# DMDung2k3/Intelligent-Video-Analysis-Retrieval-System

Measured on AMD Instinct MI355X. Metric: frames/s embedded (+ query-vs-index cosine pairs/s; top-10 recall vs CPU ref), higher is better.
Workload: dtype bf16; 1 GPU; BASELINE configs[1]: ViT-B/32 bf16 random-init embed of 224x224 RGB frames + 1M-row x 512-d fp32 index cosine top-10 (per GPU); frames_total=299008, index_rows_per_gpu=1000000, queries=10, k=10, parallelism=1 x (frames + index rows sharded per GPU); one all-gather of (score,id) + merge

## Files before the change

### intelligent-video-analysis-retrieval-system_amd/csrc/tower.hip

```cpp
#include "tower.h"
#include "tower_kernels.h"

#include <cmath>
#include <cstring>
#include <vector>

extern "C" {

int ivr_tower_create(ivr_ctx *ctx, const ivr_tower_desc *d, ivr_tower **out) {
    IVR_REQUIRE(ctx && d && out, "ivr_tower_create: NULL argument");
    IVR_REQUIRE(d->kind == IVR_KIND_VISION || d->kind == IVR_KIND_TEXT, "ivr_tower_create: kind=%d", d->kind);
    IVR_REQUIRE(d->width >= 64 && d->width % 64 == 0 && d->width <= 2048, "ivr_tower_create: width=%d must be a multiple of 64 in [64,2048]",
                d->width);
    IVR_REQUIRE(d->heads >= 1 && d->heads <= 32 && d->width == d->heads * 64, "ivr_tower_create: head_dim must be 64 (width=%d heads=%d)",
                d->width, d->heads);
    IVR_REQUIRE(d->mlp >= 64 && d->mlp % 64 == 0, "ivr_tower_create: mlp=%d must be a multiple of 64", d->mlp);
    IVR_REQUIRE(d->layers >= 1 && d->layers <= 64, "ivr_tower_create: layers=%d", d->layers);
    IVR_REQUIRE(d->tokens >= 1 && d->tokens <= 1024, "ivr_tower_create: tokens=%d", d->tokens);
    IVR_REQUIRE(d->out_dim >= 0 && d->out_dim % 16 == 0 && d->out_dim <= 2048, "ivr_tower_create: out_dim=%d", d->out_dim);
    IVR_REQUIRE(d->act == IVR_ACT_QUICK_GELU || d->act == IVR_ACT_GELU_ERF, "ivr_tower_create: act=%d", d->act);
    IVR_REQUIRE(d->compute == IVR_COMPUTE_BF16 || d->compute == IVR_COMPUTE_F32 || d->compute == IVR_COMPUTE_FP8,
                "ivr_tower_create: compute=%d", d->compute);
    IVR_REQUIRE(d->compute != IVR_COMPUTE_FP8 || (d->width % 128 == 0 && d->mlp % 128 == 0),
                "ivr_tower_create: the fp8 mode needs width and mlp to be multiples of 128 (width=%d mlp=%d)", d->width, d->mlp);
// ... 164 lines not shown
int layer_gemm(ivr_tower *t, bool site_fp8, int epi, GemmArgs &g, const std::string &wname, hipStream_t s) {
    if (site_fp8) {
        g.W = wptr<void>(t, wname + "@e4m3");
        g.colscale = wptr<float>(t, wname + "@scale");
        return ivr_launch_gemm_fp8(epi, g, s);
    }
    g.W = wptr<void>(t, wname);
    return ivr_launch_gemm(t->d.compute == IVR_COMPUTE_F32, epi, g, s);
}

int env_zigzag() {
    static const int v = [] {
        const char *e = getenv("IVR_ZIGZAG");
        return e ? (atoi(e) != 0) : 1;
    }();
    return v;
}

bool env_prune_last() {
    const char *e = getenv("IVR_PRUNE_LAST");
    return e ? (atoi(e) != 0) : true;
}

int run_layers(ivr_tower *t, int n, int T, bool prune_last, hipStream_t s) {
    const ivr_tower_desc &d = t->d;
    const bool f32 = d.compute == IVR_COMPUTE_F32;

    auto kind = [&](bool site8) { return f32 ? OUT_F32 : site8 ? OUT_FP8 : OUT_BF16; };
    const int D = d.width, rows = n * T;
    const int zz = env_zigzag();
    int rc;
    for (int i = 0; i < d.layers; ++i) {
        const std::string p = "l" + std::to_string(i) + ".";
        const int sites = i >= d.fp8_first_layer ? t->sites : 0;
        const bool q8 = sites & IVR_FP8_SITE_QKV, o8 = sites & IVR_FP8_SITE_ATTN_OUT, f18 = sites & IVR_FP8_SITE_FC1, f28 = sites & IVR_FP8_SITE_FC2;
        const bool mlp_cls = t->mlp_cls && (f18 || f28);
        const bool last = prune_last && i == d.layers - 1;
        if (t->debug_out && t->debug_layer == i)
            IVR_HIP(hipMemcpyAsync(t->debug_out, t->resid, (size_t)rows * D * 4, hipMemcpyDeviceToDevice, s));
        rc = ivr_launch_layernorm(kind(q8), t->resid, 1, nullptr, wptr<float>(t, p + "ln1_g"), wptr<float>(t, p + "ln1_b"), d.ln_eps,
                                  t->xn, rows, D, s, zz);
        if (rc) return rc;
        GemmArgs g;
        int att_ld = D;
        if (!f32 && !q8 && ivr_fused_qkv_attention_ok(rows, T, D, d.heads, d.causal)) {
            rc = ivr_launch_qkv_attention(t->xn, wptr<void>(t, p + "qkv_w"), wptr<float>(t, p + "qkv_b"), t->att, n, T, D, d.heads, o8, s, 0,
                                          last);
            if (rc) return rc;
        } else {
            if (last) att_ld = T * D;
            g.A = t->xn;
            g.lda = D;
            g.ldw = D;
            g.M = rows;
            g.N = 3 * D;
            g.K = D;
            g.bias = wptr<float>(t, p + "qkv_b");
            g.out = t->qkv;
            g.ldo = 3 * D;
            g.tag = "gemm_qkv";
            rc = layer_gemm(t, q8, EPI_STORE, g, p + "qkv_w", s);
            if (rc) return rc;
            rc = ivr_launch_attention(f32, t->qkv, t->att, n, T, D, d.heads, d.causal, s, o8);
            if (rc) return rc;
        }
        g = GemmArgs();
        g.A = t->att;
        g.lda = att_ld;
        g.ldw = D;
        g.M = last ? n : rows;
// ... 288 lines not shown
    IVR_HIP(hipSetDevice(t->ctx->device));
    hipStream_t s = (hipStream_t)stream;
    const bool f32 = d.compute == IVR_COMPUTE_F32;
    const int D = d.width, T = d.tokens, G2 = T - 1;
    int rc = ivr_launch_vision_cls(t->resid, wptr<float>(t, "cls"), wptr<float>(t, "pos"), n, T, D, s);
    if (rc) return rc;
    GemmArgs g;
    g.A = patches;
    g.lda = t->kpad;
    g.W = wptr<void>(t, "patch_w");
    g.ldw = t->kpad;
    g.M = n * G2;
    g.N = D;
    g.K = t->kpad;
    g.bias = d.patch_bias ? wptr<float>(t, "patch_b") : nullptr;
    g.resid = t->resid;
    g.ldr = D;
    g.pos = wptr<float>(t, "pos");
    g.T = T;
    g.G2 = G2;
    g.tag = "gemm_patch";
    rc = ivr_launch_gemm(f32, EPI_PATCH, g, s);
    if (rc) return rc;
    if (d.pre_ln) {
        rc = ivr_launch_layernorm(OUT_F32, t->resid, 1, nullptr, wptr<float>(t, "pre_ln_g"), wptr<float>(t, "pre_ln_b"), d.ln_eps, t->resid,
                                  n * T, D, s);
        if (rc) return rc;
    }
    const bool prune = env_prune_last() && !(t->debug_out && t->debug_layer == d.layers);
    rc = run_layers(t, n, T, prune, s);
    if (rc) return rc;
    return run_pool(t, n, T, nullptr, normalize, out, s);
}

int ivr_tower_encode_text(ivr_tower *t, const int64_t *ids, int q, int T, int normalize, float *out, ivr_stream stream) {
    IVR_REQUIRE(t && (q == 0 || (ids && out)), "ivr_tower_encode_text: NULL argument");
    std::lock_guard<std::mutex> lk(t->mu);
    if (!t->finalized) return ivr_fail(IVR_ERR_STATE, "ivr_tower_encode_text: tower not finalized");
    const ivr_tower_desc &d = t->d;
    IVR_REQUIRE(d.kind == IVR_KIND_TEXT, "ivr_tower_encode_text: not a text tower");
    IVR_REQUIRE(T >= 1 && T <= d.tokens, "ivr_tower_encode_text: T=%d outside [1,%d]", T, d.tokens);
    IVR_REQUIRE(q >= 0 && (int64_t)q * T <= (int64_t)t->max_batch * d.tokens && q <= t->max_batch,
                "ivr_tower_encode_text: q=%d exceeds max_batch=%d", q, t->max_batch);
    if (q == 0) return IVR_OK;
    IVR_HIP(hipSetDevice(t->ctx->device));
    hipStream_t s = (hipStream_t)stream;
    int rc = ivr_launch_text_embed(t->resid, ids, wptr<float>(t, "tok"), wptr<float>(t, "pos"), q, T, d.width, d.vocab, d.eos_id,
                                   t->eos_pos, s);
    if (rc) return rc;
    rc = run_layers(t, q, T, false, s);
    if (rc) return rc;
    return run_pool(t, q, T, t->eos_pos, normalize, out, s);
}
// ... 188 lines not shown
```

### intelligent-video-analysis-retrieval-system_amd/csrc/tower_kernels.h

```cpp
#pragma once
#include "ivr_common.h"

enum { EPI_STORE = 0, EPI_RESID = 1, EPI_PATCH = 2, EPI_F32 = 3 };

struct GemmArgs {
    const void *A = nullptr;
    int lda = 0;
    const void *W = nullptr;
    int ldw = 0;
    int M = 0, N = 0, K = 0;
    const float *bias = nullptr;
    void *out = nullptr;
    int ldo = 0;
    float *resid = nullptr;
    int ldr = 0;
    const float *pos = nullptr;
    int T = 0, G2 = 0;
    int act = -1;
    const char *tag = nullptr;
    int group_m = 8;
    const float *colscale = nullptr;
    int out8 = 0;
    int wide_epi = 0;
    int reverse_m = 0;
    int stagger = 0;
    int skip_mod = 0;
};

int ivr_launch_gemm(bool f32, int epi, const GemmArgs &g, hipStream_t s);
int ivr_launch_gemm_fp8(int epi, const GemmArgs &g, hipStream_t s);
enum { OUT_BF16 = 0, OUT_F32 = 1, OUT_FP8 = 2 };
int ivr_launch_layernorm(int out_kind, const float *x, int row_mul, const int *offs, const float *g, const float *b, float eps,
                         void *out, int rows, int D, hipStream_t s, int reverse = 0);
int ivr_launch_attention(bool f32, const void *qkv, void *att, int n, int T, int D, int heads, int causal, hipStream_t s,
                         bool out_fp8 = false);
bool ivr_fused_qkv_attention_shape_ok(int M, int T, int D, int heads, int causal);
bool ivr_fused_qkv_attention_ok(int M, int T, int D, int heads, int causal);
int ivr_launch_qkv_attention(const void *xn, const void *w, const float *bias, void *att, int n, int T, int D, int heads, bool out_fp8,
                             hipStream_t s, int reverse = 0, int pooled = 0);
int ivr_launch_vision_cls(float *resid, const float *cls, const float *pos, int n, int T, int D, hipStream_t s);
int ivr_launch_text_embed(float *resid, const int64_t *ids, const float *tok, const float *pos, int q, int T, int D, int vocab,
                          int eos, int *eos_pos, hipStream_t s);
int ivr_launch_bf16_to_e4m3(const void *src, void *dst, int64_t count, hipStream_t s);
int ivr_launch_f_normalize(const float *x, float *out, int n, int d, int normalize, hipStream_t s);
```

### intelligent-video-analysis-retrieval-system_amd/csrc/tower_kernels.hip

```cpp
#include "tower.h"
#include "tower_kernels.h"

#include <map>
#include <mutex>
#include <type_traits>

#include <algorithm>
#include <cstdlib>

namespace {

template <typename T>
struct El;
template <>
struct El<unsigned short> {
    static __device__ __forceinline__ void unpack(const uint4 &u, float (&f)[8]) {
        f[0] = __uint_as_float(u.x << 16);
        f[1] = __uint_as_float(u.x & 0xffff0000u);
        f[2] = __uint_as_float(u.y << 16);
        f[3] = __uint_as_float(u.y & 0xffff0000u);
        f[4] = __uint_as_float(u.z << 16);
        f[5] = __uint_as_float(u.z & 0xffff0000u);
        f[6] = __uint_as_float(u.w << 16);
        f[7] = __uint_as_float(u.w & 0xffff0000u);
// ... 81 lines not shown
__global__ __launch_bounds__(256) void text_embed_kernel(float *__restrict__ resid, const int64_t *__restrict__ ids,
                                                         const float *__restrict__ tok, const float *__restrict__ pos,
                                                         int T, int D, int vocab) {
    const int64_t r = blockIdx.x;
    const int t = (int)(r % T);
    int64_t id = ids[r];
    id = id < 0 ? 0 : (id >= vocab ? vocab - 1 : id);
    const float *e = tok + id * D;
    for (int k = threadIdx.x; k < D; k += blockDim.x) resid[r * D + k] = e[k] + pos[(int64_t)t * D + k];
}

__global__ void eos_pos_kernel(const int64_t *__restrict__ ids, int q, int T, int eos, int *__restrict__ out) {
    const int r = blockIdx.x * blockDim.x + threadIdx.x;
    if (r >= q) return;
    int p = 0;
    for (int t = 0; t < T; ++t)
        if (ids[(int64_t)r * T + t] == eos) {
            p = t;
            break;
        }
    out[r] = p;
}

template <typename TOut>
__global__ __launch_bounds__(256) void layernorm_kernel(const float *__restrict__ x, int row_mul, const int *__restrict__ offs,
                                                        const float *__restrict__ g, const float *__restrict__ b, float eps,
                                                        TOut *__restrict__ out, int rows, int D, int reverse) {
    const int lane = threadIdx.x & 63;
    int row = blockIdx.x * 4 + (threadIdx.x >> 6);
    if (row >= rows) return;
    if (reverse) row = rows - 1 - row;
    const int64_t srow = (int64_t)row * row_mul + (offs ? offs[row] : 0);
    const float4 *src = reinterpret_cast<const float4 *>(x + srow * D);
    const int nv = D >> 2;
    float4 v[8];
#pragma unroll
    for (int i = 0; i < 8; ++i) {
        const int idx = lane + 64 * i;
        v[i] = make_float4(0.f, 0.f, 0.f, 0.f);
        if (idx < nv) v[i] = src[idx];
    }
    const float x0 = __shfl(v[0].x, 0, 64);
    float s = 0.f;
#pragma unroll
    for (int i = 0; i < 8; ++i) {
        const int idx = lane + 64 * i;
        if (idx < nv) {
            v[i].x -= x0;
            v[i].y -= x0;
            v[i].z -= x0;
            v[i].w -= x0;
            s += (v[i].x + v[i].y) + (v[i].z + v[i].w);
        }
    }
    const float mean = ivr_wave_sum(s) / (float)D;
    float ss = 0.f;
#pragma unroll
    for (int i = 0; i < 8; ++i) {
        const int idx = lane + 64 * i;
        if (idx < nv) {
            const float a = v[i].x - mean, bb = v[i].y - mean, c = v[i].z - mean, d = v[i].w - mean;
            ss += (a * a + bb * bb) + (c * c + d * d);
        }
    }
    const float rstd = 1.0f / sqrtf(ivr_wave_sum(ss) / (float)D + eps);
    TOut *orow = out + (int64_t)row * D;
#pragma unroll
    for (int i = 0; i < 8; ++i) {
        const int idx = lane + 64 * i;
        if (idx < nv) {
            const float4 gg = reinterpret_cast<const float4 *>(g)[idx], bv = reinterpret_cast<const float4 *>(b)[idx];
            float y[4];
            y[0] = (v[i].x - mean) * rstd * gg.x + bv.x;
            y[1] = (v[i].y - mean) * rstd * gg.y + bv.y;
            y[2] = (v[i].z - mean) * rstd * gg.z + bv.z;
            y[3] = (v[i].w - mean) * rstd * gg.w + bv.w;
            El<TOut>::store4(orow + idx * 4, y);
        }
    }
}

__global__ __launch_bounds__(256) void f_normalize_kernel(const float *__restrict__ x, float *__restrict__ out, int n, int d,
                                                          int normalize) {
    const int lane = threadIdx.x & 63;
    const int row = blockIdx.x * 4 + (threadIdx.x >> 6);
    if (row >= n) return;
    const float *p = x + (int64_t)row * d;
    float ss = 0.f;
// ... 1235 lines not shown
                                 : "v"(offV[nt]));
                else
                    asm volatile("ds_read_b64_tr_b16 %0, %2 offset:4096\n\tds_read_b64_tr_b16 %1, %2 offset:6144\n\ts_waitcnt lgkmcnt(0)"
                                 : "=&v"(lo), "=&v"(hi)
                                 : "v"(offV[nt]));
                const uint4 vf = make_uint4(lo.x, lo.y, hi.x, hi.y);
                o = __builtin_amdgcn_mfma_f32_16x16x32_bf16(__builtin_bit_cast(bf16x8_t, vf), __builtin_bit_cast(bf16x8_t, pf[ks]), o, 0, 0, 0);
            }
            if (q < Tn) {
                const float v[4] = {o[0] * inv, o[1] * inv, o[2] * inv, o[3] * inv};
                El<TOut>::store4(op + nt * 16, v);
            }
        }
    }
}

struct QkvAttnArgs {
    const void *X = nullptr;
    const void *W = nullptr;
    const float *bias = nullptr;
    void *att = nullptr;
    int M = 0, D = 0, T = 0, heads = 0, G = 0, group_m = 4, reverse = 0;
    int pooled = 0;
};

constexpr int QA_WBYTES = 192 * ROWB;
constexpr int QA_LDS = 3 * LX_BYTES + 2 * QA_WBYTES;
constexpr int QP_LDS = 160 * 1024;
constexpr int QA_REGION = 264 * ROWB;

template <typename TOut, bool PERS>
__device__ __forceinline__ void qkv_attn_body(const QkvAttnArgs &g, unsigned char *smem) {
    typedef __bf16 bf16x8_t __attribute__((ext_vector_type(8)));
    typedef unsigned short T;
    if constexpr (!PERS) { IVR_STAMP(0) }
    const int tid = threadIdx.x, lane = tid & 63;
    const int wave = __builtin_amdgcn_readfirstlane(tid >> 6);
    const int wm = wave >> 2, wn = wave & 3;
    const int RT = g.G * g.T;
    const int MT = (g.M + RT - 1) / RT, NT = g.heads;
    const int xcd = blockIdx.x & 7, slot = blockIdx.x >> 3, nslots = gridDim.x >> 3;
    const int nitems = xcd_panels(MT, xcd) * NT;
    if (slot >= nitems) return;
    const int count = PERS ? (nitems - slot + nslots - 1) / nslots : 1;
    auto locate = [&](int n, int &tm_, int &h_) { xcd_tile(slot + n * nslots, xcd, MT, NT, g.group_m, g.reverse, tm_, h_); };
    const int KT = g.D / 64;
    const unsigned lds0 = (unsigned)(size_t)smem;

    unsigned voffX[4], voffW;
    {
        const int c = (lane & 7) ^ (lane >> 3);
#pragma unroll
        for (int j = 0; j < 4; ++j) voffX[j] = (unsigned)((8 * (wave * 4 + j) + (lane >> 3)) * g.D) * 2u + c * 16;
        voffW = (unsigned)((lane >> 3) * g.D) * 2u + c * 16;
    }
    auto item_offsets = [&](int tm_, int h_, unsigned &sx, unsigned (&sw)[3]) {
        sx = (unsigned)(tm_ * RT) * (unsigned)g.D * 2u;
#pragma unroll
        for (int j = 0; j < 3; ++j) {
            const int p = wave * 3 + j;
            sw[j] = (unsigned)(((p >> 3) * g.D + h_ * 64 + 8 * (p & 7)) * g.D) * 2u;
        }
    };
    const auto rsX = __builtin_amdgcn_make_buffer_rsrc(const_cast<void *>(g.X), 0, (int)((int64_t)g.M * g.D * 2), 0x00020000);
    const auto rsW = __builtin_amdgcn_make_buffer_rsrc(const_cast<void *>(g.W), 0, (int)((int64_t)3 * g.D * g.D * 2), 0x00020000);
    auto xbase = [](int xs) { return PERS ? (xs == 0 ? 0 : xs == 1 ? 57344 : 90112) : xs * LX_BYTES; };
    auto wbase = [](int b) { return PERS ? (b ? 122880 : 32768) : 3 * LX_BYTES + b * QA_WBYTES; };
    constexpr int IMG = PERS ? 62464 : 0;
    static_assert(IMG + 3 * QA_REGION <= (PERS ? QP_LDS : QA_LDS), "Q | K | V images past the end of the LDS");
    auto piece = [&](unsigned sx, const unsigned (&sw)[3], int kt, int xs, int j) {
        const unsigned adv = (unsigned)kt * ROWB;
        if (j < 4)
            __builtin_amdgcn_raw_ptr_buffer_load_lds(rsX, (__attribute__((address_space(3))) void *)(smem + xbase(xs) + (wave * 4 + j) * 1024), 16,
                                                     voffX[j], sx + adv, 0, 0);
        else
            __builtin_amdgcn_raw_ptr_buffer_load_lds(rsW, (__attribute__((address_space(3))) void *)(smem + wbase(kt & 1) + (wave * 3 + j - 4) * 1024),
                                                     16, voffW, sw[j - 4] + adv, 0, 0);
    };
    unsigned foX[2], foW[2];
#pragma unroll
    for (int kk = 0; kk < 2; ++kk) {
        const unsigned f = (lane & 15) * ROWB + ((((kk << 2) + (lane >> 4)) ^ (lane & 7)) << 4);
        foX[kk] = lds0 + (wm * 128) * ROWB + f;
        foW[kk] = lds0 + (wn * 48) * ROWB + f;
    }

    int tm, h;
    locate(0, tm, h);
    unsigned sx0, swW[3];
    item_offsets(tm, h, sx0, swW);
#define QA_ROW(XF, WF, MTI)                                                                                \
    _Pragma("unroll") for (int nt = 0; nt < 3; ++nt) mma_chunk<T>(WF[nt], XF[MTI], acc[nt][MTI]);          \
    __builtin_amdgcn_sched_barrier(0);
#define QA_RD3(DST, ADDR)                                                                                  \
    asm volatile("ds_read_b128 %0, %1" : "=v"(DST[0]) : "v"(ADDR));                                         \
    asm volatile("ds_read_b128 %0, %1 offset:2048" : "=v"(DST[1]) : "v"(ADDR));                             \
    asm volatile("ds_read_b128 %0, %1 offset:4096" : "=v"(DST[2]) : "v"(ADDR));

    u32x4 xa0[8], wa0[3], xa1[8], wa1[3];
    u32x4 *x0lo = xa0, *x0hi = xa0 + 4, *x1lo = xa1, *x1hi = xa1 + 4;
#pragma unroll
    for (int j = 0; j < 7; ++j) piece(sx0, swW, 0, 0, j);
  for (int n = 0; n < count; ++n) {
    const int m0 = tm * RT;
    f32x4 acc[3][8];
#pragma unroll
    for (int a = 0; a < 3; ++a)
#pragma unroll
        for (int b = 0; b < 8; ++b) acc[a][b] = f32x4{0.f, 0.f, 0.f, 0.f};
    float4 bq[3];
#pragma unroll
    for (int nt = 0; nt < 3; ++nt) {
        const int col = wn * 48 + nt * 16 + 4 * (lane >> 4);
        bq[nt] = *reinterpret_cast<const float4 *>(g.bias + (col >> 6) * g.D + h * 64 + (col & 63));
    }
#pragma unroll
    for (int j = 0; j < 7; ++j) piece(sx0, swW, 1, 1, j);
#pragma unroll
    for (int j = 0; j < 4; ++j) piece(sx0, swW, 2, 2, j);
    asm volatile("s_waitcnt vmcnt(11)\n\ts_barrier" ::: "memory");
    if constexpr (!PERS) { IVR_STAMP(1) }
    QA_RD3(wa0, foW[0] + wbase(0))
    IVR_RD4(x0lo, foX[0] + xbase(0), 0)
    IVR_RD4(x0hi, foX[0] + xbase(0), 8192)
    int xs = 0;
    for (int kt = 0; kt < KT; ++kt) {
        const int xs1 = xs == 2 ? 0 : xs + 1;
        const unsigned xoff = xbase(xs), woff = wbase(kt & 1), nxoff = xbase(xs1), nwoff = wbase((kt + 1) & 1);
        const bool tail = kt >= 1 && kt + 2 < KT;
        const bool morew = kt + 2 < KT, morex = kt + 3 < KT, next = kt + 1 < KT;
        const unsigned wa = foW[1] + woff, xa = foX[1] + xoff, nwa = foW[0] + nwoff, nxa = foX[0] + nxoff;
        IVR_LGKM(4)
        QA_ROW(xa0, wa0, 0)
        if (tail) piece(sx0, swW, kt + 2, xs1 == 2 ? 0 : xs1 + 1, 2);
        QA_ROW(xa0, wa0, 1)
        QA_RD3(wa1, wa)
        QA_ROW(xa0, wa0, 2)
        if (tail) piece(sx0, swW, kt + 2, xs1 == 2 ? 0 : xs1 + 1, 3);
        QA_ROW(xa0, wa0, 3)
        IVR_RD4(x1lo, xa, 0)
        IVR_LGKM(7)
        QA_ROW(xa0, wa0, 4)
        QA_ROW(xa0, wa0, 5)
        IVR_RD4(x1hi, xa, 8192)
        QA_ROW(xa0, wa0, 6)
        QA_ROW(xa0, wa0, 7)
        IVR_LGKM(0)
        if (next) {
            if (kt + 2 < KT) asm volatile("s_waitcnt vmcnt(4)\n\ts_barrier" ::: "memory");
            else asm volatile("s_waitcnt vmcnt(0)\n\ts_barrier" ::: "memory");
        }
        QA_ROW(xa1, wa1, 0)
        if (morew) piece(sx0, swW, kt + 2, 0, 4);
        QA_ROW(xa1, wa1, 1)
        if (next) { QA_RD3(wa0, nwa) }
        if (morew) piece(sx0, swW, kt + 2, 0, 5);
        QA_ROW(xa1, wa1, 2)
        if (morew) piece(sx0, swW, kt + 2, 0, 6);
        QA_ROW(xa1, wa1, 3)
        if (next) { IVR_RD4(x0lo, nxa, 0) }
        QA_ROW(xa1, wa1, 4)
        if (morex) piece(sx0, swW, kt + 3, xs, 0);
        QA_ROW(xa1, wa1, 5)
        if (next) { IVR_RD4(x0hi, nxa, 8192) }
        QA_ROW(xa1, wa1, 6)
        if (morex) piece(sx0, swW, kt + 3, xs, 1);
        QA_ROW(xa1, wa1, 7)
        xs = xs1;
    }
    IVR_LGKM(0)
#undef QA_ROW
#undef QA_RD3
    if constexpr (!PERS) { IVR_STAMP(2) }
    __builtin_amdgcn_s_barrier();

    unsigned char *const qreg = smem + IMG, *const kreg = smem + IMG + QA_REGION, *const vreg = smem + IMG + 2 * QA_REGION;
    {
        const int r = lane & 15, gq = lane >> 4;
#pragma unroll
        for (int nt = 0; nt < 3; ++nt) {
            const int col = wn * 48 + nt * 16 + 4 * gq;
            const int reg3 = col >> 6, dh = col & 63, ch = dh >> 3;
            const float4 bv = bq[nt];
            unsigned char *base = smem + IMG + reg3 * QA_REGION + (dh & 7) * 2;
#pragma unroll
            for (int mt = 0; mt < 8; ++mt) {
                const int m = wm * 128 + mt * 16 + r;
                const f32x4 a = acc[nt][mt];
                uint2 o;
                o.x = ivr_pack_bf16x2(a[0] + bv.x, a[1] + bv.y);
                o.y = ivr_pack_bf16x2(a[2] + bv.z, a[3] + bv.w);
                const unsigned pos = reg3 == 2 ? (unsigned)((((ch >> 1) ^ ((m >> 1) & 3)) << 5) | ((ch & 1) << 4))
                                               : (unsigned)((ch ^ (m & 7)) << 4);
                *reinterpret_cast<uint2 *>(base + m * ROWB + pos) = o;
            }
        }
        if (tid < 128) *reinterpret_cast<uint4 *>((tid < 64 ? kreg : vreg) + 256 * ROWB + (tid & 63) * 16) = make_uint4(0u, 0u, 0u, 0u);
    }
    __syncthreads();
#ifdef IVR_GEMM_STAMPS
    if (!PERS && threadIdx.x == 0 && blockIdx.x < 16384) ivr_gemm_stamps[blockIdx.x][6] = __builtin_amdgcn_s_memtime();
#endif
    const int h_cur = h;
    if (n + 1 < count) {
        locate(n + 1, tm, h);
        item_offsets(tm, h, sx0, swW);
#pragma unroll
        for (int j = 0; j < 7; ++j) piece(sx0, swW, 0, 0, j);
    }

    const int Tn = g.T, nqt = g.pooled ? 1 : (Tn + 15) >> 4, units = g.G * nqt;
    const int gl = lane >> 4, c = lane & 15;
    constexpr float L2E = 1.4426950408889634f;
    for (int u = wave; u < units; u += 8) {
        const int img = u / nqt, qt = u - img * nqt;
        const int R0 = img * Tn;
        if (m0 + R0 >= g.M) continue;
        const int q = qt * 16 + c;
        uint4 qf[2], kf[2][4];
        uint2 vt[4][4];
        {
            const int rq = R0 + q;
            const unsigned qa = (unsigned)(size_t)qreg + rq * ROWB, qx = rq & 7;
#pragma unroll
            for (int ks = 0; ks < 2; ++ks) asm volatile("ds_read_b128 %0, %1" : "=v"(qf[ks]) : "v"(qa + (((4 * ks + gl) ^ qx) << 4)));
            const int rk = R0 + c;
            const unsigned ka = (unsigned)(size_t)kreg + rk * ROWB, kx = rk & 7;
#pragma unroll
            for (int ks = 0; ks < 2; ++ks) {
                const unsigned a0 = ka + (((4 * ks + gl) ^ kx) << 4);
                asm volatile("ds_read_b128 %0, %1" : "=v"(kf[ks][0]) : "v"(a0));
// ... 84 lines not shown
        }
    }
    if (n + 1 < count) __syncthreads();
  }
#ifdef IVR_GEMM_STAMPS
    if constexpr (!PERS) {
        asm volatile("s_waitcnt vmcnt(0)" ::: "memory");
        __syncthreads();
        IVR_STAMP(3)
    }
#endif
}

template <typename TOut>
__global__ __launch_bounds__(512, 2) void qkv_attn_kernel(QkvAttnArgs g) {
    extern __shared__ __attribute__((aligned(16))) unsigned char smem[];
    qkv_attn_body<TOut, false>(g, smem);
}

template <typename TOut>
__global__ __launch_bounds__(512, 2) void qkv_attn_pers_kernel(QkvAttnArgs g) {
    extern __shared__ __attribute__((aligned(16))) unsigned char smem[];
    qkv_attn_body<TOut, true>(g, smem);
}

template <int EPI, int ACT>
__global__ __launch_bounds__(512, 2) void gemm_pers_kernel(GemmArgs g) {
    typedef unsigned short T;
    extern __shared__ __attribute__((aligned(16))) unsigned char smem[];
    const int tid = threadIdx.x, lane = tid & 63;
    const int wave = __builtin_amdgcn_readfirstlane(tid >> 6);
    const int wm = wave >> 2, wn = wave & 3;
    const int MT = (g.M + LBM - 1) / LBM, NT = (g.N + LBN - 1) / LBN;
    const int xcd = blockIdx.x & 7, slot = blockIdx.x >> 3, nslots = gridDim.x >> 3;
    const int lx = MT > xcd ? (MT - xcd + 7) >> 3 : 0;
    const int nitems = lx * NT;
    if (slot >= nitems) return;
    const int count = (nitems - slot + nslots - 1) / nslots;
    const int KT = g.K / 64;
    const int S = count * KT;
    const unsigned lds0 = (unsigned)(size_t)smem;
    const int gm = g.group_m;
    auto locate = [&](int n, int &tm, int &tn) {
        const unsigned i = (unsigned)(slot + n * nslots);
        const unsigned per = (unsigned)(gm * NT), grp = i / per, within = i - grp * per;
        const unsigned gme = (unsigned)min(gm, lx - (int)grp * gm);
// ... 501 lines not shown
        if (g.act == IVR_ACT_GELU_ERF) return launch_gemm8_t<EPI_STORE, IVR_ACT_GELU_ERF, true>(g, s);
        return launch_gemm8_t<EPI_STORE, -1, true>(g, s);
    }
    if (g.act == IVR_ACT_QUICK_GELU) return launch_gemm8_t<EPI_STORE, IVR_ACT_QUICK_GELU, false>(g, s);
    if (g.act == IVR_ACT_GELU_ERF) return launch_gemm8_t<EPI_STORE, IVR_ACT_GELU_ERF, false>(g, s);
    return launch_gemm8_t<EPI_STORE, -1, false>(g, s);
}

bool ivr_fused_qkv_attention_shape_ok(int M, int T, int D, int heads, int causal) {
    if (T < 1 || T > 64 || causal || D % 64 != 0 || D < 192 || D > 2048 || heads != D / 64 || M < 0 || M % T != 0) return false;
    return (int64_t)M * D * 2 < 0x7fffffff && (int64_t)3 * D * D * 2 < 0x7fffffff;
}

bool ivr_fused_qkv_attention_ok(int M, int T, int D, int heads, int causal) {
    if (!ivr_fused_qkv_attention_shape_ok(M, T, D, heads, causal)) return false;
    const int mode = env_int("IVR_FUSED_QKV", -1);
    if (mode == 0) return false;
    if (mode == 1) return true;
    const int RT = (256 / T) * T;
    return (int64_t)((M + RT - 1) / RT) * heads >= 256;
}

int ivr_launch_qkv_attention(const void *xn, const void *w, const float *bias, void *att, int n, int T, int D, int heads, bool out_fp8,
                             hipStream_t s, int reverse, int pooled) {
    if (n <= 0) return IVR_OK;
    const int M = n * T;
    IVR_REQUIRE(ivr_fused_qkv_attention_shape_ok(M, T, D, heads, 0), "fused qkv+attention: unsupported shape (n=%d T=%d D=%d heads=%d)",
                n, T, D, heads);
    const auto al16 = [](const void *p) { return reinterpret_cast<uintptr_t>(p) % 16 == 0; };
    IVR_REQUIRE(al16(xn) && al16(w) && al16(bias) && al16(att), "fused qkv+attention: operands must be 16-byte aligned");
    QkvAttnArgs g;
    g.X = xn;
    g.W = w;
    g.bias = bias;
    g.att = att;
    g.M = M;
    g.D = D;
    g.T = T;
    g.heads = heads;
    g.G = 256 / T;
    g.group_m = std::max(1, env_int("IVR_QKV_GROUP_M", 4));
    g.reverse = reverse;
    g.pooled = pooled != 0;
    const int RT = g.G * T, MT = (M + RT - 1) / RT;
    IvrProf prof("gemm_qkv_attention", s, 2.0 * M * 3.0 * D * D + 4.0 * n * heads * (double)(pooled ? std::min(T, 16) : T) * T * 64);
    const int qpers = env_int("IVR_QKV_PERS", 1);
    const bool pers = qpers == 2 || (qpers == 1 && (int64_t)MT * heads >= 2 * device_cu_count());
    void (*kern)(QkvAttnArgs) = pers ? (out_fp8 ? qkv_attn_pers_kernel<unsigned char> : qkv_attn_pers_kernel<unsigned short>)
                                     : (out_fp8 ? qkv_attn_kernel<unsigned char> : qkv_attn_kernel<unsigned short>);
    const int grid = pers ? device_cu_count() / 8 * 8 : xcd_grid(MT, heads), lds = pers ? QP_LDS : QA_LDS;
    if (int rc = ivr_func_max_lds(reinterpret_cast<const void *>(kern), lds)) return rc;
    hipLaunchKernelGGL(kern, dim3(grid), dim3(512), lds, s, g);
    IVR_LAUNCH_CHECK();
    return IVR_OK;
}

int ivr_launch_layernorm(int out_kind, const float *x, int row_mul, const int *offs, const float *g, const float *b, float eps,
                         void *out, int rows, int D, hipStream_t s, int reverse) {
    if (rows <= 0) return IVR_OK;
    IVR_REQUIRE(D % 4 == 0 && D <= 2048, "layernorm: D=%d", D);
    const unsigned grid = (unsigned)ivr_ceil_div(rows, 4);
    IvrProf prof("layernorm", s, (double)rows * D * (4 + (out_kind == OUT_F32 ? 4 : out_kind == OUT_FP8 ? 1 : 2)));
    if (out_kind == OUT_F32)
        hipLaunchKernelGGL(layernorm_kernel<float>, dim3(grid), dim3(256), 0, s, x, row_mul, offs, g, b, eps, (float *)out, rows, D, reverse);
    else if (out_kind == OUT_FP8)
        hipLaunchKernelGGL(layernorm_kernel<unsigned char>, dim3(grid), dim3(256), 0, s, x, row_mul, offs, g, b, eps,
                           (unsigned char *)out, rows, D, reverse);
    else
        hipLaunchKernelGGL(layernorm_kernel<unsigned short>, dim3(grid), dim3(256), 0, s, x, row_mul, offs, g, b, eps,
                           (unsigned short *)out, rows, D, reverse);
    IVR_LAUNCH_CHECK();
    return IVR_OK;
}

int ivr_launch_attention(bool f32, const void *qkv, void *att, int n, int T, int D, int heads, int causal, hipStream_t s, bool out_fp8) {
    if (n <= 0) return IVR_OK;
    IvrProf prof("attention", s, 4.0 * n * heads * (double)T * T * 64);
    IVR_REQUIRE(!(f32 && out_fp8), "attention: e4m3 output only from the bf16 kernels");
    if (!f32 && T <= 64) {
        const int64_t items = (int64_t)n * heads;
        if (out_fp8)
            hipLaunchKernelGGL(attention_mfma_short_kernel<unsigned char>, dim3((unsigned)ivr_ceil_div(items, 4)), dim3(256), 4 * 8192,
                               s, (const unsigned short *)qkv, (unsigned char *)att, n, T, D, heads, causal);
        else
            hipLaunchKernelGGL(attention_mfma_short_kernel<unsigned short>, dim3((unsigned)ivr_ceil_div(items, 4)), dim3(256), 4 * 8192,
                               s, (const unsigned short *)qkv, (unsigned short *)att, n, T, D, heads, causal);
        IVR_LAUNCH_CHECK();
        return IVR_OK;
    }
    if (!f32) {
        const int Tp = (int)ivr_round_up(T, 32);
        const int head_env = env_int("IVR_ATTN_HEAD", 1);
        if (head_env && 2 * Tp * 128 <= 160 * 1024 && (int64_t)T * 3 * D * 2 < 0x7fffffff) {
            const int ntiles = (T + 15) / 16;
            auto go = [&](auto qc_c, auto minw_c) -> int {
// ... 126 lines not shown
```

Measured before the change: 105,300 frames/s.

## Fuse pre-LN with layer-0 LN1 and skip full Q projection in pruned last layer

Adds a chained layernorm kernel that applies pre_ln, writes the fp32 residual back in place, and then applies layer 0's ln1 to produce xn, all in one launch, so the separate pre_ln pass and its extra read of the residual go away. In the pruned last layer, only CLS-row queries are needed. A small GEMM now projects Q for just those rows, and a new NOQ variant of the fused qkv+attention kernel computes only K and V and loads the precomputed Q rows into LDS. This cuts roughly a third of the QKV GEMM work in the last layer, at the cost of an extra small GEMM launch, more kernel variants, and tighter wait counts that could be fragile.

```diff
diff --git a/intelligent-video-analysis-retrieval-system_amd/csrc/tower.hip b/intelligent-video-analysis-retrieval-system_amd/csrc/tower.hip
--- a/intelligent-video-analysis-retrieval-system_amd/csrc/tower.hip
+++ b/intelligent-video-analysis-retrieval-system_amd/csrc/tower.hip
@@ -210,7 +210,22 @@
     return e ? (atoi(e) != 0) : true;
 }
 
-int run_layers(ivr_tower *t, int n, int T, bool prune_last, hipStream_t s) {
+bool env_preln_fused() {
+    const char *e = getenv("IVR_PRELN_FUSED");
+    return e ? (atoi(e) != 0) : true;
+}
+
+bool env_last_noq() {
+    const char *e = getenv("IVR_LAST_NOQ");
+    return e ? (atoi(e) != 0) : true;
+}
+
+int site_kind(const ivr_tower *t, int layer, int bit) {
+    const int sites = layer >= t->d.fp8_first_layer ? t->sites : 0;
+    return t->d.compute == IVR_COMPUTE_F32 ? OUT_F32 : (sites & bit) ? OUT_FP8 : OUT_BF16;
+}
+
+int run_layers(ivr_tower *t, int n, int T, bool prune_last, hipStream_t s, bool ln1_done = false) {
     const ivr_tower_desc &d = t->d;
     const bool f32 = d.compute == IVR_COMPUTE_F32;
 
@@ -226,14 +241,32 @@
         const bool last = prune_last && i == d.layers - 1;
         if (t->debug_out && t->debug_layer == i)
             IVR_HIP(hipMemcpyAsync(t->debug_out, t->resid, (size_t)rows * D * 4, hipMemcpyDeviceToDevice, s));
-        rc = ivr_launch_layernorm(kind(q8), t->resid, 1, nullptr, wptr<float>(t, p + "ln1_g"), wptr<float>(t, p + "ln1_b"), d.ln_eps,
-                                  t->xn, rows, D, s, zz);
-        if (rc) return rc;
+        if (!(ln1_done && i == 0)) {
+            rc = ivr_launch_layernorm(kind(q8), t->resid, 1, nullptr, wptr<float>(t, p + "ln1_g"), wptr<float>(t, p + "ln1_b"), d.ln_eps,
+                                      t->xn, rows, D, s, zz);
+            if (rc) return rc;
+        }
         GemmArgs g;
         int att_ld = D;
         if (!f32 && !q8 && ivr_fused_qkv_attention_ok(rows, T, D, d.heads, d.causal)) {
+            const void *qrow = nullptr;
+            if (last && env_last_noq()) {
+                g.A = t->xn;
+                g.lda = T * D;
+                g.ldw = D;
+                g.M = n;
+                g.N = D;
+                g.K = D;
+                g.bias = wptr<float>(t, p + "qkv_b");
+                g.out = t->qkv;
+                g.ldo = D;
+                g.tag = "gemm_q_cls";
+                rc = layer_gemm(t, false, EPI_STORE, g, p + "qkv_w", s);
+                if (rc) return rc;
+                qrow = t->qkv;
+            }
             rc = ivr_launch_qkv_attention(t->xn, wptr<void>(t, p + "qkv_w"), wptr<float>(t, p + "qkv_b"), t->att, n, T, D, d.heads, o8, s, 0,
-                                          last);
+                                          last, qrow);
             if (rc) return rc;
         } else {
             if (last) att_ld = T * D;
@@ -568,13 +601,19 @@
     g.tag = "gemm_patch";
     rc = ivr_launch_gemm(f32, EPI_PATCH, g, s);
     if (rc) return rc;
-    if (d.pre_ln) {
+    const bool preln_fused = d.pre_ln && env_preln_fused();
+    if (preln_fused) {
+        rc = ivr_launch_layernorm2(site_kind(t, 0, IVR_FP8_SITE_QKV), t->resid, wptr<float>(t, "pre_ln_g"), wptr<float>(t, "pre_ln_b"),
+                                   d.ln_eps, wptr<float>(t, "l0.ln1_g"), wptr<float>(t, "l0.ln1_b"), d.ln_eps, t->xn, n * T, D, s,
+                                   env_zigzag());
+        if (rc) return rc;
+    } else if (d.pre_ln) {
         rc = ivr_launch_layernorm(OUT_F32, t->resid, 1, nullptr, wptr<float>(t, "pre_ln_g"), wptr<float>(t, "pre_ln_b"), d.ln_eps, t->resid,
                                   n * T, D, s);
         if (rc) return rc;
     }
     const bool prune = env_prune_last() && !(t->debug_out && t->debug_layer == d.layers);
-    rc = run_layers(t, n, T, prune, s);
+    rc = run_layers(t, n, T, prune, s, preln_fused);
     if (rc) return rc;
     return run_pool(t, n, T, nullptr, normalize, out, s);
 }
diff --git a/intelligent-video-analysis-retrieval-system_amd/csrc/tower_kernels.h b/intelligent-video-analysis-retrieval-system_amd/csrc/tower_kernels.h
--- a/intelligent-video-analysis-retrieval-system_amd/csrc/tower_kernels.h
+++ b/intelligent-video-analysis-retrieval-system_amd/csrc/tower_kernels.h
@@ -32,12 +32,14 @@
 enum { OUT_BF16 = 0, OUT_F32 = 1, OUT_FP8 = 2 };
 int ivr_launch_layernorm(int out_kind, const float *x, int row_mul, const int *offs, const float *g, const float *b, float eps,
                          void *out, int rows, int D, hipStream_t s, int reverse = 0);
+int ivr_launch_layernorm2(int out_kind, float *x, const float *g, const float *b, float eps, const float *g2, const float *b2, float eps2,
+                          void *out, int rows, int D, hipStream_t s, int reverse = 0);
 int ivr_launch_attention(bool f32, const void *qkv, void *att, int n, int T, int D, int heads, int causal, hipStream_t s,
                          bool out_fp8 = false);
 bool ivr_fused_qkv_attention_shape_ok(int M, int T, int D, int heads, int causal);
 bool ivr_fused_qkv_attention_ok(int M, int T, int D, int heads, int causal);
 int ivr_launch_qkv_attention(const void *xn, const void *w, const float *bias, void *att, int n, int T, int D, int heads, bool out_fp8,
-                             hipStream_t s, int reverse = 0, int pooled = 0);
+                             hipStream_t s, int reverse = 0, int pooled = 0, const void *qrow = nullptr);
 int ivr_launch_vision_cls(float *resid, const float *cls, const float *pos, int n, int T, int D, hipStream_t s);
 int ivr_launch_text_embed(float *resid, const int64_t *ids, const float *tok, const float *pos, int q, int T, int D, int vocab,
                           int eos, int *eos_pos, hipStream_t s);
diff --git a/intelligent-video-analysis-retrieval-system_amd/csrc/tower_kernels.hip b/intelligent-video-analysis-retrieval-system_amd/csrc/tower_kernels.hip
--- a/intelligent-video-analysis-retrieval-system_amd/csrc/tower_kernels.hip
+++ b/intelligent-video-analysis-retrieval-system_amd/csrc/tower_kernels.hip
@@ -127,10 +127,38 @@
     out[r] = p;
 }
 
-template <typename TOut>
-__global__ __launch_bounds__(256) void layernorm_kernel(const float *__restrict__ x, int row_mul, const int *__restrict__ offs,
+__device__ __forceinline__ void ln_row_stats(float4 (&v)[8], int lane, int nv, int D, float eps, float &mean, float &rstd) {
+    const float x0 = __shfl(v[0].x, 0, 64);
+    float s = 0.f;
+#pragma unroll
+    for (int i = 0; i < 8; ++i) {
+        const int idx = lane + 64 * i;
+        if (idx < nv) {
+            v[i].x -= x0;
+            v[i].y -= x0;
+            v[i].z -= x0;
+            v[i].w -= x0;
+            s += (v[i].x + v[i].y) + (v[i].z + v[i].w);
+        }
+    }
+    mean = ivr_wave_sum(s) / (float)D;
+    float ss = 0.f;
+#pragma unroll
+    for (int i = 0; i < 8; ++i) {
+        const int idx = lane + 64 * i;
+        if (idx < nv) {
+            const float a = v[i].x - mean, bb = v[i].y - mean, c = v[i].z - mean, d = v[i].w - mean;
+            ss += (a * a + bb * bb) + (c * c + d * d);
+        }
+    }
+    rstd = 1.0f / sqrtf(ivr_wave_sum(ss) / (float)D + eps);
+}
+
+template <typename TOut, bool CHAIN = false>
+__global__ __launch_bounds__(256) void layernorm_kernel(const float *x, int row_mul, const int *__restrict__ offs,
                                                         const float *__restrict__ g, const float *__restrict__ b, float eps,
-                                                        TOut *__restrict__ out, int rows, int D, int reverse) {
+                                                        float *mid, const float *__restrict__ g2, const float *__restrict__ b2,
+                                                        float eps2, TOut *__restrict__ out, int rows, int D, int reverse) {
     const int lane = threadIdx.x & 63;
     int row = blockIdx.x * 4 + (threadIdx.x >> 6);
     if (row >= rows) return;
@@ -145,30 +173,26 @@
         v[i] = make_float4(0.f, 0.f, 0.f, 0.f);
         if (idx < nv) v[i] = src[idx];
     }
-    const float x0 = __shfl(v[0].x, 0, 64);
-    float s = 0.f;
-#pragma unroll
-    for (int i = 0; i < 8; ++i) {
-        const int idx = lane + 64 * i;
-        if (idx < nv) {
-            v[i].x -= x0;
-            v[i].y -= x0;
-            v[i].z -= x0;
-            v[i].w -= x0;
-            s += (v[i].x + v[i].y) + (v[i].z + v[i].w);
-        }
-    }
-    const float mean = ivr_wave_sum(s) / (float)D;
-    float ss = 0.f;
-#pragma unroll
-    for (int i = 0; i < 8; ++i) {
-        const int idx = lane + 64 * i;
-        if (idx < nv) {
-            const float a = v[i].x - mean, bb = v[i].y - mean, c = v[i].z - mean, d = v[i].w - mean;
-            ss += (a * a + bb * bb) + (c * c + d * d);
-        }
-    }
-    const float rstd = 1.0f / sqrtf(ivr_wave_sum(ss) / (float)D + eps);
+    float mean, rstd;
+    ln_row_stats(v, lane, nv, D, eps, mean, rstd);
+    if constexpr (CHAIN) {
+        float4 *mrow = reinterpret_cast<float4 *>(mid + (int64_t)row * D);
+#pragma unroll
+        for (int i = 0; i < 8; ++i) {
+            const int idx = lane + 64 * i;
+            if (idx < nv) {
+                const float4 gg = reinterpret_cast<const float4 *>(g)[idx], bv = reinterpret_cast<const float4 *>(b)[idx];
+                v[i].x = (v[i].x - mean) * rstd * gg.x + bv.x;
+                v[i].y = (v[i].y - mean) * rstd * gg.y + bv.y;
+                v[i].z = (v[i].z - mean) * rstd * gg.z + bv.z;
+                v[i].w = (v[i].w - mean) * rstd * gg.w + bv.w;
+                mrow[idx] = v[i];
+            }
+        }
+        ln_row_stats(v, lane, nv, D, eps2, mean, rstd);
+        g = g2;
+        b = b2;
+    }
     TOut *orow = out + (int64_t)row * D;
 #pragma unroll
     for (int i = 0; i < 8; ++i) {
@@ -1450,6 +1474,7 @@
     void *att = nullptr;
     int M = 0, D = 0, T = 0, heads = 0, G = 0, group_m = 4, reverse = 0;
     int pooled = 0;
+    const void *qrow = nullptr;
 };
 
 constexpr int QA_WBYTES = 192 * ROWB;
@@ -1457,8 +1482,10 @@
 constexpr int QP_LDS = 160 * 1024;
 constexpr int QA_REGION = 264 * ROWB;
 
-template <typename TOut, bool PERS>
+template <typename TOut, bool PERS, bool NOQ = false>
 __device__ __forceinline__ void qkv_attn_body(const QkvAttnArgs &g, unsigned char *smem) {
+    constexpr int NT3 = NOQ ? 2 : 3;
+    constexpr int REG0 = NOQ ? 1 : 0;
     typedef __bf16 bf16x8_t __attribute__((ext_vector_type(8)));
     typedef unsigned short T;
     if constexpr (!PERS) { IVR_STAMP(0) }
@@ -1482,12 +1509,12 @@
         for (int j = 0; j < 4; ++j) voffX[j] = (unsigned)((8 * (wave * 4 + j) + (lane >> 3)) * g.D) * 2u + c * 16;
         voffW = (unsigned)((lane >> 3) * g.D) * 2u + c * 16;
     }
-    auto item_offsets = [&](int tm_, int h_, unsigned &sx, unsigned (&sw)[3]) {
+    auto item_offsets = [&](int tm_, int h_, unsigned &sx, unsigned (&sw)[NT3]) {
         sx = (unsigned)(tm_ * RT) * (unsigned)g.D * 2u;
 #pragma unroll
-        for (int j = 0; j < 3; ++j) {
-            const int p = wave * 3 + j;
-            sw[j] = (unsigned)(((p >> 3) * g.D + h_ * 64 + 8 * (p & 7)) * g.D) * 2u;
+        for (int j = 0; j < NT3; ++j) {
+            const int p = wave * NT3 + j;
+            sw[j] = (unsigned)(((REG0 + (p >> 3)) * g.D + h_ * 64 + 8 * (p & 7)) * g.D) * 2u;
         }
     };
     const auto rsX = __builtin_amdgcn_make_buffer_rsrc(const_cast<void *>(g.X), 0, (int)((int64_t)g.M * g.D * 2), 0x00020000);
@@ -1496,13 +1523,13 @@
     auto wbase = [](int b) { return PERS ? (b ? 122880 : 32768) : 3 * LX_BYTES + b * QA_WBYTES; };
     constexpr int IMG = PERS ? 62464 : 0;
     static_assert(IMG + 3 * QA_REGION <= (PERS ? QP_LDS : QA_LDS), "Q | K | V images past the end of the LDS");
-    auto piece = [&](unsigned sx, const unsigned (&sw)[3], int kt, int xs, int j) {
+    auto piece = [&](unsigned sx, const unsigned (&sw)[NT3], int kt, int xs, int j) {
         const unsigned adv = (unsigned)kt * ROWB;
         if (j < 4)
             __builtin_amdgcn_raw_ptr_buffer_load_lds(rsX, (__attribute__((address_space(3))) void *)(smem + xbase(xs) + (wave * 4 + j) * 1024), 16,
                                                      voffX[j], sx + adv, 0, 0);
         else
-            __builtin_amdgcn_raw_ptr_buffer_load_lds(rsW, (__attribute__((address_space(3))) void *)(smem + wbase(kt & 1) + (wave * 3 + j - 4) * 1024),
+            __builtin_amdgcn_raw_ptr_buffer_load_lds(rsW, (__attribute__((address_space(3))) void *)(smem + wbase(kt & 1) + (wave * NT3 + j - 4) * 1024),
                                                      16, voffW, sw[j - 4] + adv, 0, 0);
     };
     unsigned foX[2], foW[2];
@@ -1510,43 +1537,43 @@
     for (int kk = 0; kk < 2; ++kk) {
         const unsigned f = (lane & 15) * ROWB + ((((kk << 2) + (lane >> 4)) ^ (lane & 7)) << 4);
         foX[kk] = lds0 + (wm * 128) * ROWB + f;
-        foW[kk] = lds0 + (wn * 48) * ROWB + f;
+        foW[kk] = lds0 + (wn * 16 * NT3) * ROWB + f;
     }
 
     int tm, h;
     locate(0, tm, h);
-    unsigned sx0, swW[3];
+    unsigned sx0, swW[NT3];
     item_offsets(tm, h, sx0, swW);
 #define QA_ROW(XF, WF, MTI)                                                                                \
-    _Pragma("unroll") for (int nt = 0; nt < 3; ++nt) mma_chunk<T>(WF[nt], XF[MTI], acc[nt][MTI]);          \
+    _Pragma("unroll") for (int nt = 0; nt < NT3; ++nt) mma_chunk<T>(WF[nt], XF[MTI], acc[nt][MTI]);        \
     __builtin_amdgcn_sched_barrier(0);
 #define QA_RD3(DST, ADDR)                                                                                  \
     asm volatile("ds_read_b128 %0, %1" : "=v"(DST[0]) : "v"(ADDR));                                         \
     asm volatile("ds_read_b128 %0, %1 offset:2048" : "=v"(DST[1]) : "v"(ADDR));                             \
-    asm volatile("ds_read_b128 %0, %1 offset:4096" : "=v"(DST[2]) : "v"(ADDR));
+    if constexpr (!NOQ) asm volatile("ds_read_b128 %0, %1 offset:4096" : "=v"(DST[2]) : "v"(ADDR));
 
     u32x4 xa0[8], wa0[3], xa1[8], wa1[3];
     u32x4 *x0lo = xa0, *x0hi = xa0 + 4, *x1lo = xa1, *x1hi = xa1 + 4;
 #pragma unroll
-    for (int j = 0; j < 7; ++j) piece(sx0, swW, 0, 0, j);
+    for (int j = 0; j < 4 + NT3; ++j) piece(sx0, swW, 0, 0, j);
   for (int n = 0; n < count; ++n) {
     const int m0 = tm * RT;
-    f32x4 acc[3][8];
-#pragma unroll
-    for (int a = 0; a < 3; ++a)
+    f32x4 acc[NT3][8];
+#pragma unroll
+    for (int a = 0; a < NT3; ++a)
 #pragma unroll
         for (int b = 0; b < 8; ++b) acc[a][b] = f32x4{0.f, 0.f, 0.f, 0.f};
-    float4 bq[3];
-#pragma unroll
-    for (int nt = 0; nt < 3; ++nt) {
-        const int col = wn * 48 + nt * 16 + 4 * (lane >> 4);
-        bq[nt] = *reinterpret_cast<const float4 *>(g.bias + (col >> 6) * g.D + h * 64 + (col & 63));
-    }
-#pragma unroll
-    for (int j = 0; j < 7; ++j) piece(sx0, swW, 1, 1, j);
+    float4 bq[NT3];
+#pragma unroll
+    for (int nt = 0; nt < NT3; ++nt) {
+        const int col = wn * 16 * NT3 + nt * 16 + 4 * (lane >> 4);
+        bq[nt] = *reinterpret_cast<const float4 *>(g.bias + (REG0 + (col >> 6)) * g.D + h * 64 + (col & 63));
+    }
+#pragma unroll
+    for (int j = 0; j < 4 + NT3; ++j) piece(sx0, swW, 1, 1, j);
 #pragma unroll
     for (int j = 0; j < 4; ++j) piece(sx0, swW, 2, 2, j);
-    asm volatile("s_waitcnt vmcnt(11)\n\ts_barrier" ::: "memory");
+    wait_vm_barrier<8 + NT3>();
     if constexpr (!PERS) { IVR_STAMP(1) }
     QA_RD3(wa0, foW[0] + wbase(0))
     IVR_RD4(x0lo, foX[0] + xbase(0), 0)
@@ -1567,7 +1594,7 @@
         if (tail) piece(sx0, swW, kt + 2, xs1 == 2 ? 0 : xs1 + 1, 3);
         QA_ROW(xa0, wa0, 3)
         IVR_RD4(x1lo, xa, 0)
-        IVR_LGKM(7)
+        if constexpr (NOQ) { IVR_LGKM(6) } else { IVR_LGKM(7) }
         QA_ROW(xa0, wa0, 4)
         QA_ROW(xa0, wa0, 5)
         IVR_RD4(x1hi, xa, 8192)
@@ -1584,7 +1611,8 @@
         if (next) { QA_RD3(wa0, nwa) }
         if (morew) piece(sx0, swW, kt + 2, 0, 5);
         QA_ROW(xa1, wa1, 2)
-        if (morew) piece(sx0, swW, kt + 2, 0, 6);
+        if constexpr (!NOQ)
+            if (morew) piece(sx0, swW, kt + 2, 0, 6);
         QA_ROW(xa1, wa1, 3)
         if (next) { IVR_RD4(x0lo, nxa, 0) }
         QA_ROW(xa1, wa1, 4)
@@ -1606,9 +1634,9 @@
     {
         const int r = lane & 15, gq = lane >> 4;
 #pragma unroll
-        for (int nt = 0; nt < 3; ++nt) {
-            const int col = wn * 48 + nt * 16 + 4 * gq;
-            const int reg3 = col >> 6, dh = col & 63, ch = dh >> 3;
+        for (int nt = 0; nt < NT3; ++nt) {
+            const int col = wn * 16 * NT3 + nt * 16 + 4 * gq;
+            const int reg3 = REG0 + (col >> 6), dh = col & 63, ch = dh >> 3;
             const float4 bv = bq[nt];
             unsigned char *base = smem + IMG + reg3 * QA_REGION + (dh & 7) * 2;
 #pragma unroll
@@ -1624,6 +1652,14 @@
             }
         }
         if (tid < 128) *reinterpret_cast<uint4 *>((tid < 64 ? kreg : vreg) + 256 * ROWB + (tid & 63) * 16) = make_uint4(0u, 0u, 0u, 0u);
+        if constexpr (NOQ) {
+            for (int i = tid; i < g.G * 8; i += 512) {
+                const int img = i >> 3, chq = i & 7, m = img * g.T;
+                if (m0 + m < g.M)
+                    *reinterpret_cast<uint4 *>(qreg + m * ROWB + ((chq ^ (m & 7)) << 4)) = *reinterpret_cast<const uint4 *>(
+                        reinterpret_cast<const unsigned short *>(g.qrow) + (int64_t)(m0 / g.T + img) * g.D + h * 64 + chq * 8);
+            }
+        }
     }
     __syncthreads();
 #ifdef IVR_GEMM_STAMPS
@@ -1634,7 +1670,7 @@
         locate(n + 1, tm, h);
         item_offsets(tm, h, sx0, swW);
 #pragma unroll
-        for (int j = 0; j < 7; ++j) piece(sx0, swW, 0, 0, j);
+        for (int j = 0; j < 4 + NT3; ++j) piece(sx0, swW, 0, 0, j);
     }
 
     const int Tn = g.T, nqt = g.pooled ? 1 : (Tn + 15) >> 4, units = g.G * nqt;
@@ -1765,6 +1801,18 @@
 __global__ __launch_bounds__(512, 2) void qkv_attn_pers_kernel(QkvAttnArgs g) {
     extern __shared__ __attribute__((aligned(16))) unsigned char smem[];
     qkv_attn_body<TOut, true>(g, smem);
+}
+
+template <typename TOut>
+__global__ __launch_bounds__(512, 2) void qkv_attn_noq_kernel(QkvAttnArgs g) {
+    extern __shared__ __attribute__((aligned(16))) unsigned char smem[];
+    qkv_attn_body<TOut, false, true>(g, smem);
+}
+
+template <typename TOut>
+__global__ __launch_bounds__(512, 2) void qkv_attn_pers_noq_kernel(QkvAttnArgs g) {
+    extern __shared__ __attribute__((aligned(16))) unsigned char smem[];
+    qkv_attn_body<TOut, true, true>(g, smem);
 }
 
 template <int EPI, int ACT>
@@ -2312,13 +2360,14 @@
 }
 
 int ivr_launch_qkv_attention(const void *xn, const void *w, const float *bias, void *att, int n, int T, int D, int heads, bool out_fp8,
-                             hipStream_t s, int reverse, int pooled) {
+                             hipStream_t s, int reverse, int pooled, const void *qrow) {
     if (n <= 0) return IVR_OK;
     const int M = n * T;
     IVR_REQUIRE(ivr_fused_qkv_attention_shape_ok(M, T, D, heads, 0), "fused qkv+attention: unsupported shape (n=%d T=%d D=%d heads=%d)",
                 n, T, D, heads);
     const auto al16 = [](const void *p) { return reinterpret_cast<uintptr_t>(p) % 16 == 0; };
-    IVR_REQUIRE(al16(xn) && al16(w) && al16(bias) && al16(att), "fused qkv+attention: operands must be 16-byte aligned");
+    IVR_REQUIRE(al16(xn) && al16(w) && al16(bias) && al16(att) && al16(qrow), "fused qkv+attention: operands must be 16-byte aligned");
+    IVR_REQUIRE(!qrow || pooled, "fused qkv+attention: projected Q rows only with the pooled mode");
     QkvAttnArgs g;
     g.X = xn;
     g.W = w;
@@ -2332,12 +2381,17 @@
     g.group_m = std::max(1, env_int("IVR_QKV_GROUP_M", 4));
     g.reverse = reverse;
     g.pooled = pooled != 0;
+    g.qrow = qrow;
     const int RT = g.G * T, MT = (M + RT - 1) / RT;
-    IvrProf prof("gemm_qkv_attention", s, 2.0 * M * 3.0 * D * D + 4.0 * n * heads * (double)(pooled ? std::min(T, 16) : T) * T * 64);
+    IvrProf prof("gemm_qkv_attention", s,
+                 2.0 * M * (qrow ? 2.0 : 3.0) * D * D + 4.0 * n * heads * (double)(pooled ? std::min(T, 16) : T) * T * 64);
     const int qpers = env_int("IVR_QKV_PERS", 1);
     const bool pers = qpers == 2 || (qpers == 1 && (int64_t)MT * heads >= 2 * device_cu_count());
-    void (*kern)(QkvAttnArgs) = pers ? (out_fp8 ? qkv_attn_pers_kernel<unsigned char> : qkv_attn_pers_kernel<unsigned short>)
-                                     : (out_fp8 ? qkv_attn_kernel<unsigned char> : qkv_attn_kernel<unsigned short>);
+    void (*kern)(QkvAttnArgs) =
+        qrow ? (pers ? (out_fp8 ? qkv_attn_pers_noq_kernel<unsigned char> : qkv_attn_pers_noq_kernel<unsigned short>)
+                     : (out_fp8 ? qkv_attn_noq_kernel<unsigned char> : qkv_attn_noq_kernel<unsigned short>))
+             : (pers ? (out_fp8 ? qkv_attn_pers_kernel<unsigned char> : qkv_attn_pers_kernel<unsigned short>)
+                     : (out_fp8 ? qkv_attn_kernel<unsigned char> : qkv_attn_kernel<unsigned short>));
     const int grid = pers ? device_cu_count() / 8 * 8 : xcd_grid(MT, heads), lds = pers ? QP_LDS : QA_LDS;
     if (int rc = ivr_func_max_lds(reinterpret_cast<const void *>(kern), lds)) return rc;
     hipLaunchKernelGGL(kern, dim3(grid), dim3(512), lds, s, g);
@@ -2345,22 +2399,36 @@
     return IVR_OK;
 }
 
-int ivr_launch_layernorm(int out_kind, const float *x, int row_mul, const int *offs, const float *g, const float *b, float eps,
-                         void *out, int rows, int D, hipStream_t s, int reverse) {
+namespace {
+template <bool CHAIN>
+int launch_layernorm_t(int out_kind, const float *x, int row_mul, const int *offs, const float *g, const float *b, float eps, float *mid,
+                       const float *g2, const float *b2, float eps2, void *out, int rows, int D, hipStream_t s, int reverse) {
     if (rows <= 0) return IVR_OK;
     IVR_REQUIRE(D % 4 == 0 && D <= 2048, "layernorm: D=%d", D);
     const unsigned grid = (unsigned)ivr_ceil_div(rows, 4);
-    IvrProf prof("layernorm", s, (double)rows * D * (4 + (out_kind == OUT_F32 ? 4 : out_kind == OUT_FP8 ? 1 : 2)));
+    IvrProf prof("layernorm", s, (double)rows * D * ((CHAIN ? 8 : 4) + (out_kind == OUT_F32 ? 4 : out_kind == OUT_FP8 ? 1 : 2)));
     if (out_kind == OUT_F32)
-        hipLaunchKernelGGL(layernorm_kernel<float>, dim3(grid), dim3(256), 0, s, x, row_mul, offs, g, b, eps, (float *)out, rows, D, reverse);
+        hipLaunchKernelGGL((layernorm_kernel<float, CHAIN>), dim3(grid), dim3(256), 0, s, x, row_mul, offs, g, b, eps, mid, g2, b2, eps2,
+                           (float *)out, rows, D, reverse);
     else if (out_kind == OUT_FP8)
-        hipLaunchKernelGGL(layernorm_kernel<unsigned char>, dim3(grid), dim3(256), 0, s, x, row_mul, offs, g, b, eps,
-                           (unsigned char *)out, rows, D, reverse);
+        hipLaunchKernelGGL((layernorm_kernel<unsigned char, CHAIN>), dim3(grid), dim3(256), 0, s, x, row_mul, offs, g, b, eps, mid, g2, b2,
+                           eps2, (unsigned char *)out, rows, D, reverse);
     else
-        hipLaunchKernelGGL(layernorm_kernel<unsigned short>, dim3(grid), dim3(256), 0, s, x, row_mul, offs, g, b, eps,
-                           (unsigned short *)out, rows, D, reverse);
+        hipLaunchKernelGGL((layernorm_kernel<unsigned short, CHAIN>), dim3(grid), dim3(256), 0, s, x, row_mul, offs, g, b, eps, mid, g2, b2,
+                           eps2, (unsigned short *)out, rows, D, reverse);
     IVR_LAUNCH_CHECK();
     return IVR_OK;
+}
+}
+
+int ivr_launch_layernorm(int out_kind, const float *x, int row_mul, const int *offs, const float *g, const float *b, float eps,
+                         void *out, int rows, int D, hipStream_t s, int reverse) {
+    return launch_layernorm_t<false>(out_kind, x, row_mul, offs, g, b, eps, nullptr, nullptr, nullptr, 0.f, out, rows, D, s, reverse);
+}
+
+int ivr_launch_layernorm2(int out_kind, float *x, const float *g, const float *b, float eps, const float *g2, const float *b2, float eps2,
+                          void *out, int rows, int D, hipStream_t s, int reverse) {
+    return launch_layernorm_t<true>(out_kind, x, 1, nullptr, g, b, eps, x, g2, b2, eps2, out, rows, D, s, reverse);
 }
 
 int ivr_launch_attention(bool f32, const void *qkv, void *att, int n, int T, int D, int heads, int causal, hipStream_t s, bool out_fp8) {
```

Result: no change. 106,000 frames/s, median of 6 (+0.6%).
